# evanwporter/SparseCholesky

Hardware: AMD Instinct MI355X
Metric: numeric-factorization fp64 GFLOP/s (F=sum colcount^2) (higher is better)
Workload: dtype f64

## Files before the change

sparsecholesky_amd/csrc/kernels.hip:

```cpp
#include <hip/hip_runtime.h>

#include <cstdint>
#include <type_traits>

#include "kernels.hpp"

namespace sc {

typedef double double4_t __attribute__((ext_vector_type(4)));

__device__ __forceinline__ void report_fail(int32_t* info, const int32_t* post, int32_t col_internal) {
    atomicMin(info, (post ? post[col_internal] : col_internal) + 1);
}

__device__ __forceinline__ int bnd_at(const int32_t* b, int k, int mbc) {
    const int klo = b[0], khi = b[1];
    return k <= klo ? b[2] : (k >= khi ? mbc : b[2 + k - klo]);
}

__device__ __forceinline__ int lower_bound_i32(const int32_t* a, int n, int v) {
    int lo = 0, hi = n;
    while (lo < hi) {
        int mid = (lo + hi) >> 1;
        if (a[mid] < v)
// ... 677 lines not shown
        }
    }
}

template <int NP, int J>
__device__ __forceinline__ void td_steps(double (&a)[NP], double (&Ld)[4][4], double (&rc)[4], int& bad, int& fail,
                                         double* raw, double* lv, int i) {
    if constexpr (J < NP) {
        __builtin_amdgcn_sched_barrier(0);
        if (bad < 4) fail = min(fail, J + bad);
        const bool below = i >= J + 4;
        double l[4];
#pragma unroll
        for (int k = 0; k < 4; ++k) {
            double x = below ? a[J + k] : 0.0;
#pragma unroll
            for (int t = 0; t < k; ++t) x = fma(-l[t], Ld[k][t], x);
            l[k] = x * rc[k];
        }
        wave_lds_sync();
        *reinterpret_cast<double2*>(lv + 4 * i) = make_double2(l[0], l[1]);
        *reinterpret_cast<double2*>(lv + 4 * i + 2) = make_double2(l[2], l[3]);
        wave_lds_sync();
#pragma unroll
        for (int c = 0; c < 4; ++c) {
            double v = below ? l[c] : a[J + c];
#pragma unroll
            for (int r = c; r < 4; ++r) v = i == J + r ? Ld[r][c] : v;
            a[J + c] = v;
        }
        auto update = [&](int jj) {
            const double2 x01 = *reinterpret_cast<const double2*>(lv + 4 * jj);
            const double2 x23 = *reinterpret_cast<const double2*>(lv + 4 * jj + 2);
            double x = a[jj];
            x = fma(-l[0], x01.x, x);
            x = fma(-l[1], x01.y, x);
            x = fma(-l[2], x23.x, x);
            x = fma(-l[3], x23.y, x);
            a[jj] = x;
        };
        if constexpr (J + 4 < NP && !SC_TD_LA) {
#pragma unroll
            for (int jj = J + 4; jj < NP; ++jj) update(jj);
            wave_lds_sync();
            *reinterpret_cast<double2*>(raw + 4 * i) = make_double2(a[J + 4], a[J + 5]);
            *reinterpret_cast<double2*>(raw + 4 * i + 2) = make_double2(a[J + 6], a[J + 7]);
            wave_lds_sync();
            td_factor_d(raw, J + 4, Ld, rc, bad);
        }
        if constexpr (J + 4 < NP && SC_TD_LA) {
#pragma unroll
            for (int jj = J + 4; jj < J + 8; ++jj) update(jj);
            wave_lds_sync();
            *reinterpret_cast<double2*>(raw + 4 * i) = make_double2(a[J + 4], a[J + 5]);
            *reinterpret_cast<double2*>(raw + 4 * i + 2) = make_double2(a[J + 6], a[J + 7]);
            wave_lds_sync();
            double Dn[4][4], Ln[4][4], rn[4];
            int bn = 4;
#pragma unroll
            for (int r = 0; r < 4; ++r) {
                const double2 x01 = *reinterpret_cast<const double2*>(raw + 4 * (J + 4 + r));
                const double2 x23 = *reinterpret_cast<const double2*>(raw + 4 * (J + 4 + r) + 2);
                Dn[r][0] = x01.x;
                Dn[r][1] = x01.y;
                Dn[r][2] = x23.x;
                Dn[r][3] = x23.y;
            }
            auto pivot = [&](int c) {
                double dd = Dn[c][c];
#pragma unroll
                for (int t = 0; t < c; ++t) dd = fma(-Ln[c][t], Ln[c][t], dd);
                if (!(dd > 0.0)) bn = min(bn, c);
                rn[c] = rsqrt_f64(dd);
                Ln[c][c] = dd * rn[c];
#pragma unroll
                for (int r = c + 1; r < 4; ++r) {
                    double x = Dn[r][c];
#pragma unroll
                    for (int t = 0; t < c; ++t) x = fma(-Ln[r][t], Ln[c][t], x);
                    Ln[r][c] = x * rn[c];
                }
            };
            constexpr int GW = NP > 48 ? 4 : 8;
            constexpr int NG = (NP - J - 8 + GW - 1) / GW;
#pragma unroll
            for (int g = 0; g < NG; ++g) {
                if (g < 4) pivot(g);
#pragma unroll
                for (int u = 0; u < GW; ++u)
                    if (J + 8 + GW * g + u < NP) update(J + 8 + GW * g + u);
                __builtin_amdgcn_sched_barrier(0);
            }
#pragma unroll
            for (int c = NG; c < 4; ++c) pivot(c);
#pragma unroll
            for (int r = 0; r < 4; ++r) {
                rc[r] = rn[r];
#pragma unroll
                for (int c = 0; c < 4; ++c) Ld[r][c] = Ln[r][c];
            }
            bad = bn;
        }
        td_steps<NP, J + 4>(a, Ld, rc, bad, fail, raw, lv, i);
    }
}

template <int NP>
__global__ __launch_bounds__(64) void tiny_dense_kernel(DevPlan P, TinyPlan T, int n, const double* __restrict__ Ax) {
    __shared__ __attribute__((aligned(16))) double raw[NP * 4];
    __shared__ __attribute__((aligned(16))) double lv[NP * 4];
    __shared__ int po[NP * 64];
    const int i = threadIdx.x;
    int2 q[NP];
#pragma unroll
    for (int j = 0; j < NP; ++j) q[j] = T.a[j * 64 + i];
#pragma unroll
    for (int j = 0; j < NP; ++j) po[j * 64 + i] = q[j].y;
    double a[NP];
    int fail = n;
    double Ld[4][4], rc[4];
    int bad;
#pragma unroll
    for (int j = 0; j < NP; ++j) {
#if SC_TD_BUF
        a[j] = buf_ld(buf_rsrc(Ax, (uint32_t)T.nax * 8u), q[j].x >= 0 ? q[j].x * 8 : BUF_DEAD, 0);
#else
        a[j] = q[j].x >= 0 ? Ax[q[j].x] : 0.0;
#endif
    }
#pragma unroll
    for (int j = 0; j < NP; ++j) a[j] = (i == j && i >= n) ? 1.0 : a[j];
    if (SC_TD_PROBE != 1) {
        wave_lds_sync();
        *reinterpret_cast<double2*>(raw + 4 * i) = make_double2(a[0], a[1]);
        *reinterpret_cast<double2*>(raw + 4 * i + 2) = make_double2(a[2], a[3]);
        wave_lds_sync();
        td_factor_d(raw, 0, Ld, rc, bad);
        td_steps<NP, 0>(a, Ld, rc, bad, fail, raw, lv, i);
    }
    if (fail > n) fail = n;
#pragma unroll
    for (int j = 0; j < NP; ++j) {
        const int o = po[j * 64 + i];
#if SC_TD_BUF
        buf_st(a[j], buf_rsrc(P.panel_pool, (uint32_t)T.npan * 8u), o >= 0 ? o * 8 : BUF_DEAD, 0);
#else
        if (o >= 0) P.panel_pool[o] = a[j];
#endif
    }
    int32_t nat = fail < n ? (P.post ? P.post[fail] : fail) : 0x7f7f7f7f;
    if (fail < n) {
        __shared__ double rec[NP * 64];
#pragma unroll
        for (int j = 0; j < NP; ++j) {
            const int2 q = T.a[j * 64 + i];
            rec[j * 64 + i] = q.x >= 0 ? Ax[q.x] : 0.0;
        }
        for (int j = 0; j < n; ++j) {
            wave_lds_sync();
            const double d = rec[j * 64 + j];
            const bool ok = d > 0.0;
            if (!ok) nat = min(nat, P.post ? P.post[j] : j);
            const double l = (ok && i > j) ? rec[j * 64 + i] / sqrt(d) : 0.0;
            lv[i] = l;
            wave_lds_sync();
            for (int k = j + 1; k < n; ++k)
                if (i >= k) rec[k * 64 + i] -= l * lv[k];
        }
    }
    if (i == 0) {
        if (T.host_info) {
            const int32_t st = fail < n ? nat + 1 : 0x7f7f7f7f;
            P.info[0] = st;
            __hip_atomic_store(T.host_info, st, __ATOMIC_RELEASE, __HIP_MEMORY_SCOPE_SYSTEM);
        } else if (fail < n) {
            atomicMin(P.info, nat + 1);
        }
    }
}

hipError_t launch_tiny_dense(const DevPlan& P, const TinyPlan& T, int n, const double* Ax, hipStream_t st) {
    if (n <= 0) return hipSuccess;
    if (n > TINY_DENSE_N || T.na != tiny_dense_np(n) * 64) return hipErrorInvalidValue;
    if ((int64_t)T.nax * 8 >= BUF_DEAD || (int64_t)T.npan * 8 >= BUF_DEAD) return hipErrorInvalidValue;
    if (n <= 16)
        hipLaunchKernelGGL(tiny_dense_kernel<16>, dim3(1), dim3(64), 0, st, P, T, n, Ax);
    else if (n <= 32)
        hipLaunchKernelGGL(tiny_dense_kernel<32>, dim3(1), dim3(64), 0, st, P, T, n, Ax);
    else if (n <= 48)
        hipLaunchKernelGGL(tiny_dense_kernel<48>, dim3(1), dim3(64), 0, st, P, T, n, Ax);
    else
        hipLaunchKernelGGL(tiny_dense_kernel<64>, dim3(1), dim3(64), 0, st, P, T, n, Ax);
    return hipGetLastError();
}

__global__ __launch_bounds__(256) void chain_init_kernel(DevPlan P, ChainPlan C, int first,
                                                          const double* __restrict__ Ax) {
    extern __shared__ double F[];
    const ChainDesc d = C.desc[first + blockIdx.x];
    small_assemble(P, d.s, d.c0, d.w, d.m, Ax, F, d.sp);
    const int tot = (d.m * (d.m + 1)) >> 1;
    double* out = C.init + d.init_off;
    for (int idx = threadIdx.x; idx < tot; idx += 256) out[idx] = F[idx];
}

#ifndef SC_CHAIN_DB
#define SC_CHAIN_DB 1
#endif
constexpr int CHAIN_IMG = (128 * 129 / 2 + CHAIN_NT - 1) / CHAIN_NT;
__global__ __launch_bounds__(CHAIN_NT) void front_chain_kernel(DevPlan P, ChainPlan C, int first, int count, int fsz) {
    extern __shared__ double F[];
    __shared__ __attribute__((aligned(16))) double colbuf[2 * 4 * COLB];
    __shared__ ChainDesc ds[CHAIN_MAXF];
    const int tid = threadIdx.x;
    for (int i = tid; i < count; i += CHAIN_NT) ds[i] = C.desc[first + i];
    lds_barrier();
    double img[CHAIN_IMG];
    int nbi, nbj;
    uint32_t nrr, nrc;
    auto prefetch = [&](int f) {
        const ChainDesc& d = ds[f];
        const int tot = (d.m * (d.m + 1)) >> 1;
        const double* src = C.init + d.init_off;
#pragma unroll
        for (int q = 0; q < CHAIN_IMG; ++q) {
            const int idx = tid + CHAIN_NT * q;
            img[q] = idx < tot ? src[idx] : 0.0;
        }
        const int T = (d.m + 3) >> 2;
        nbi = nbj = -1;
        if (tid < T * (T + 1) / 2) tile_map(tid, T, (d.w + 3) >> 2, nbi, nbj);
        nrr = nbi >= 0 ? C.relp[d.relp_off + nbi] : 0u;
        nrc = nbi >= 0 ? C.relp[d.relp_off + nbj] : 0u;
    };
    auto Fb = [&](int f) { return SC_CHAIN_DB ? F + (f & 1) * fsz : F; };
    auto put = [&](int f) {
        const int tot = (ds[f].m * (ds[f].m + 1)) >> 1;
        double* Fd = Fb(f);
#pragma unroll
        for (int q = 0; q < CHAIN_IMG; ++q) {
            const int idx = tid + CHAIN_NT * q;
            if (idx < tot) Fd[idx] = img[q];
        }
    };
    int cbi, cbj;
    uint32_t crr, crc;
    auto take = [&]() {
        cbi = nbi;
        cbj = nbj;
        crr = nrr;
        crc = nrc;
    };
    prefetch(0);
    put(0);
    take();
    if (count > 1) prefetch(1);
    lds_barrier();
    for (int i = 0; i < count; ++i) {
        uint64_t* stamp = C.stamps ? C.stamps + 8 * (first + i) : nullptr;
        if (stamp && tid == 0) stamp[0] = __builtin_amdgcn_s_memtime();
        const ChainDesc d = ds[i];
        const int m = d.m, w = d.w;
        SmallRegs<1> R;
        R.bi[0] = cbi;
        R.bj[0] = cbj;
        const uint32_t rr = crr, rc = crc;
        small_load<1>(R, Fb(i), m);
        if (!SC_CHAIN_DB) lds_barrier();
        if (stamp && tid == 0) stamp[1] = __builtin_amdgcn_s_memtime();
        const bool has_parent = i + 1 < count;
        if (has_parent) {
            put(i + 1);
            take();
            if (i + 2 < count) prefetch(i + 2);
        }
        if (stamp && tid == 0) stamp[2] = __builtin_amdgcn_s_memtime();
        small_steps<1>(R, colbuf, w, P.info, P.post, d.c0);
        if (w == 0) lds_barrier();
        if (stamp && tid == 0) stamp[3] = __builtin_amdgcn_s_memtime();
        small_store_panel<1>(R, P.panel_pool + d.panel_off, m, w);
        if (m > w && R.bi[0] >= 0 && 4 * R.bi[0] + 3 >= w) {
            if (!has_parent) {
                small_store_cb<1>(R, P.cb_pool + d.cb_off, m, w);
            } else {
                const int mp = ds[i + 1].m;
                double* Fp = Fb(i + 1);
#pragma unroll
                for (int r = 0; r < 4; ++r)
#pragma unroll
                    for (int c = 0; c < 4; ++c) {
                        const int ii = 4 * R.bi[0] + r, jj = 4 * R.bj[0] + c;
                        const int pr = (rr >> (8 * r)) & 255, pc = (rc >> (8 * c)) & 255;
                        if (jj >= w && ii >= jj && ii < m) Fp[pk_col(mp, pc) + pr - pc] += R.v[0][r * 4 + c];
                    }
            }
        }
        lds_barrier();
        if (stamp && tid == 0) stamp[4] = __builtin_amdgcn_s_memtime();
    }
}

#include "panel_gen.inc"

__global__ __launch_bounds__(256) void potrf_tiles_kernel(DevPlan P, const int2* __restrict__ tasks) {
    __shared__ __attribute__((aligned(16))) double colbuf[2 * 4 * COLB];
    const int2 t = tasks[blockIdx.x];
    const int s = t.x, k0 = t.y;
    const int c0 = P.sn_start[s];
    const int w = P.sn_start[s + 1] - c0;
    const int m = P.sn_m[s];
    const int nb = min(PNB, w - k0);
    double* blk = P.panel_pool + P.panel_off[s] + (int64_t)k0 * m + k0;
    SmallRegs<1> R;
    small_tiles<1>(R, nb, nb);
#pragma unroll
    for (int r = 0; r < 4; ++r)
#pragma unroll
        for (int c = 0; c < 4; ++c) {
            const int i = 4 * R.bi[0] + r, j = 4 * R.bj[0] + c;
            R.v[0][r * 4 + c] = (R.bi[0] >= 0 && i < nb && i >= j) ? blk[(int64_t)j * m + i] : 0.0;
        }
    if (SC_POTRF_FAST)
        small_steps1_fast(R, colbuf, nb, P.info, P.post, c0 + k0);
    else
        small_steps<1>(R, colbuf, nb, P.info, P.post, c0 + k0);
    if (R.bi[0] < 0) return;
#pragma unroll
    for (int r = 0; r < 4; ++r)
#pragma unroll
        for (int c = 0; c < 4; ++c) {
            const int i = 4 * R.bi[0] + r, j = 4 * R.bj[0] + c;
            if (i < nb && i >= j) blk[(int64_t)j * m + i] = R.v[0][r * 4 + c];
        }
}

__device__ __forceinline__ void trsm_partial(double* pan, int m, int k0, int nb, int r0, int nrows, double* Lc,
                                             double* invd) {
    constexpr int LD = PNB + 2;
    const int tid = threadIdx.x;
    const double* blk = pan + (int64_t)k0 * m + k0;
    for (int idx = tid; idx < PNB * PNB; idx += TRSM_ROWS) {
        const int q = idx % PNB, j = idx / PNB;
        const double v = (q < nb && j < nb && j <= q) ? blk[(int64_t)j * m + q] : 0.0;
        Lc[j * LD + q] = v;
        if (q == j) invd[j] = (j < nb) ? 1.0 / v : 0.0;
    }
    __syncthreads();
    const int row = r0 + tid;
    const bool live = row < m && tid < nrows;
    double* xs = pan + (int64_t)k0 * m + (live ? row : r0);
    double r[PNB];
#pragma unroll
    for (int c = 0; c < PNB; ++c) r[c] = (live && c < nb) ? xs[(int64_t)c * m] : 0.0;
    trsm_steps<0>(r, Lc, invd, nb);
    if (live) {
#pragma unroll
        for (int c = 0; c < PNB; ++c)
            if (c < nb) xs[(int64_t)c * m] = r[c];
    }
}

__global__ __launch_bounds__(TRSM_ROWS) void trsm_partial_kernel(DevPlan P, const TrsmTask* __restrict__ tasks) {
    __shared__ double Lc[PNB * (PNB + 2)];
    __shared__ double invd[PNB];
    const TrsmTask t = tasks[blockIdx.x];
    const int s = t.s, k0 = t.k0, r0 = t.r0;
    const int c0 = P.sn_start[s];
    const int w = P.sn_start[s + 1] - c0;
    const int m = P.sn_m[s];
    trsm_partial(P.panel_pool + P.panel_off[s], m, k0, min(PNB, w - k0), r0, min(TRSM_ROWS, t.r1 - r0), Lc, invd);
}

template <int PRE>
__global__ __launch_bounds__(TRSM_ROWS) void trsm_panel_g_kernel(DevPlan P, const TrsmTask* __restrict__ tasks,
                                                                 int32_t* __restrict__ arrive) {
    static_assert(TRSM_ROWS == 256, "the fused POTRF maps 4 x 4 tiles onto 256 threads");
    __shared__ double2 S[TRSM64_STREAM / 2];
    __shared__ __attribute__((aligned(16))) double colbuf[2 * 4 * COLB];
    __shared__ int s_last;
    const TrsmTask t = tasks[blockIdx.x];
    const int s = t.s, k0 = t.k0, r0 = t.r0, r1 = t.r1;
    const int tid = threadIdx.x;
    const int c0 = P.sn_start[s];
    const int w = P.sn_start[s + 1] - c0;
    const int m = P.sn_m[s];
    const int nb = min(PNB, w - k0);
    double* pan = P.panel_pool + P.panel_off[s];
    if (nb < PNB) return;
    double* blk = pan + (int64_t)k0 * m + k0;
    double* Sd = reinterpret_cast<double*>(S);
    SmallRegs<1> R;
    small_tiles<1>(R, PNB, PNB);
#pragma unroll
    for (int r = 0; r < 4; ++r)
#pragma unroll
        for (int c = 0; c < 4; ++c) {
            const int i = 4 * R.bi[0] + r, j = 4 * R.bj[0] + c;
            R.v[0][r * 4 + c] = (R.bi[0] >= 0 && i >= j) ? blk[(int64_t)j * m + i] : 0.0;
        }
    if constexpr (PRE == 2) {
        if (R.bi[0] >= 0) {
#pragma unroll
            for (int r = 0; r < 4; ++r)
#pragma unroll
                for (int c = 0; c < 4; ++c) {
                    const int i = 4 * R.bi[0] + r, j = 4 * R.bj[0] + c;
                    if (i >= j) Sd[PNB * j - j * (j - 1) / 2 + (i - j)] = (i == j) ? 1.0 / R.v[0][r * 4 + c] : R.v[0][r * 4 + c];
                }
        }
        const int row = r0 + tid;
        const __amdgpu_buffer_rsrc_t rs = buf_rsrc(pan + (int64_t)k0 * m, (uint32_t)m * PNB * 8u);
        const int voff = row < r1 ? row * 8 : BUF_DEAD;
        double r[PNB];
#pragma unroll
        for (int c = 0; c < PNB; ++c) r[c] = buf_ld(rs, voff, c * m * 8);
        __syncthreads();
        trsm64_full(r, S);
#pragma unroll
        for (int c = 0; c < PNB; ++c) buf_st(r[c], rs, voff, c * m * 8);
        return;
    }
    if (SC_POTRF_FAST)
        small_steps1_fast(R, colbuf, PNB, P.info, P.post, c0 + k0);
    else
        small_steps<1>(R, colbuf, PNB, P.info, P.post, c0 + k0);
    if (R.bi[0] >= 0) {
#pragma unroll
        for (int r = 0; r < 4; ++r)
#pragma unroll
            for (int c = 0; c < 4; ++c) {
                const int i = 4 * R.bi[0] + r, j = 4 * R.bj[0] + c;
                if (i >= j) Sd[PNB * j - j * (j - 1) / 2 + (i - j)] = (i == j) ? 1.0 / R.v[0][r * 4 + c] : R.v[0][r * 4 + c];
            }
    }
    const int row = r0 + tid;
    const __amdgpu_buffer_rsrc_t rs = buf_rsrc(pan + (int64_t)k0 * m, (uint32_t)m * PNB * 8u);
    const int voff = row < r1 ? row * 8 : BUF_DEAD;
    double r[PNB];
#pragma unroll
    for (int c = 0; c < PNB; ++c) r[c] = buf_ld(rs, voff, c * m * 8);
    __syncthreads();
    if (tid == 0) {
        const int k1 = k0 + PNB;
        const int nwg = (max(r1, k1 + 1) - k1 + TRSM_ROWS - 1) / TRSM_ROWS;
        const int old = __hip_atomic_fetch_add(arrive + (t.ctr - 1), 1, __ATOMIC_RELAXED, __HIP_MEMORY_SCOPE_AGENT);
        s_last = old == nwg - 1;
        if (old == nwg - 1) __hip_atomic_store(arrive + (t.ctr - 1), 0, __ATOMIC_RELAXED, __HIP_MEMORY_SCOPE_AGENT);
    }
    __syncthreads();
    if (s_last && R.bi[0] >= 0) {
#pragma unroll
        for (int rr = 0; rr < 4; ++rr)
#pragma unroll
            for (int c = 0; c < 4; ++c) {
                const int i = 4 * R.bi[0] + rr, j = 4 * R.bj[0] + c;
                if (i >= j) blk[(int64_t)j * m + i] = R.v[0][rr * 4 + c];
            }
    }
    trsm64_full(r, S);
#pragma unroll
    for (int c = 0; c < PNB; ++c) buf_st(r[c], rs, voff, c * m * 8);
}

#ifndef SC_PROBE_NOGATHER
#define SC_PROBE_NOGATHER 0
#endif
#ifndef SC_PROBE_NOK
#define SC_PROBE_NOK 0
#endif
template <int BT, int WM, int WN, int BK = 16, int GR = 64>
__device__ __forceinline__ void syrk_gather_epilogue(const GemmTask& T, const int64_t* __restrict__ gblk,
                                                     const GSeg* __restrict__ gseg, int row0, int col0,
                                                     double4_t (&acc)[BT / WM / 16][BT / WN / 16], double* smem) {
    constexpr int NW = WM * WN, NT = 64 * NW;
    constexpr int RTM = BT / WM / 16, RTN = BT / WN / 16;
    constexpr int GLD = GR + 1;
    constexpr int GQ = BT == 64 ? (GR == 32 ? 8 : 64 / NW) : SC_GATHER_Q;
    constexpr int SB = BT == 64 ? 4 : 1;
    constexpr int OPS = 2 * 2 * BK * (BT + 16);
    static_assert(BT * GLD <= OPS, "gather chunk fits the operand LDS");
    const int tid = threadIdx.x, lane = tid & 63, wid = tid >> 6;
    const int wr = wid / WN, wc = wid % WN;
    const int w = T.gw;
    const int mb = T.M;
    const int nb = (mb + 63) >> 6;
    const int64_t* __restrict__ blk = gblk + T.gb;
    const GSeg* __restrict__ seg = gseg;
    double* G = smem;
    double* __restrict__ C = T.C;
    const int64_t ldc = T.ldc;
    const __amdgpu_buffer_rsrc_t rc = buf_rsrc(C + (int64_t)col0 * ldc, (uint32_t)(min(BT, T.N - col0) * ldc * 8));
#pragma unroll 1
    for (int h = 0; h < BT / GR; ++h) {
        const int r0 = row0 + h * GR;
        const int rb = r0 >> 6;
        if (h) __syncthreads();
        for (int e = tid; e < BT * GLD; e += NT) G[e] = 0.0;
        __syncthreads();
        const int cb1 = min(min(nb, rb + 1), (col0 + BT) >> 6);
        for (int cbk = col0 >> 6; !SC_PROBE_NOGATHER && r0 < mb && cbk < cb1; ++cbk) {
            const int64_t bi = (int64_t)rb * (rb + 1) / 2 + cbk;
            const int64_t p0 = blk[bi], p1 = blk[bi + 1];
            for (int64_t pb = p0; pb < p1; pb += SB) {
                int prw[SB], pcl[SB];
#pragma unroll
                for (int q = 0; q < SB; ++q) {
                    prw[q] = -1;
                    pcl[q] = -1;
                    if (pb + q < p1) {
                        const GSeg& g = seg[pb + q];
                        const int ic = g.ilo + lane, jl = g.jlo + lane;
                        if (ic < g.ihi) prw[q] = g.rel[ic] - w - r0;
                        if (jl < g.jhi) pcl[q] = g.rel[jl] - w - col0;
                    }
                }
#pragma unroll
                for (int q = 0; q < SB; ++q) {
                    if (pb + q >= p1) break;
                    const GSeg& g = seg[pb + q];
                    const int ic = g.ilo + lane;
                    const int prow = prw[q] < GR ? prw[q] : -1;
                    const int mbc = g.mbc;
                    const double* __restrict__ cb = g.cb;
                    uint64_t mask = __ballot(pcl[q] >= 0 && pcl[q] % NW == wid);
                    while (mask) {
                        int jc[GQ], pc[GQ];
#pragma unroll
                        for (int u = 0; u < GQ; ++u) {
                            const int b = mask ? __builtin_ctzll(mask) : -1;
                            jc[u] = b < 0 ? -1 : g.jlo + b;
                            pc[u] = b < 0 ? 0 : __builtin_amdgcn_readlane(pcl[q], b);
                            mask &= mask - 1;
                        }
                        double v[GQ];
                        bool ok[GQ];
#pragma unroll
                        for (int u = 0; u < GQ; ++u) {
                            ok[u] = jc[u] >= 0 && prow >= 0 && ic >= jc[u];
                            const __amdgpu_buffer_rsrc_t rs = buf_rsrc(cb + (int64_t)max(jc[u], 0) * mbc, (uint32_t)mbc * 8u);
                            v[u] = buf_ld(rs, ok[u] ? ic * 8 : BUF_DEAD, 0);
                        }
#pragma unroll
                        for (int u = 0; u < GQ; ++u)
                            if (ok[u]) G[pc[u] * GLD + prow] += v[u];
                    }
                }
            }
        }
        __syncthreads();
        static_assert(GR % (BT / WM) == 0, "a wave's rows lie in one chunk");
        if ((wr * (BT / WM)) / GR == h) {
#pragma unroll
            for (int a = 0; a < RTM; ++a)
#pragma unroll
                for (int b = 0; b < RTN; ++b)
#pragma unroll
                    for (int r = 0; r < 4; ++r) {
                        const int lr = wr * (BT / WM) + a * 16 + MFMA_F64_ROW(lane, r);
                        const int lc = wc * (BT / WN) + b * 16 + (lane & 15);
                        G[lc * GLD + (lr - h * GR)] -= acc[a][b][r];
                    }
        }
        __syncthreads();
#pragma unroll 4
        for (int e = tid; e < BT * GR; e += NT) {
            const int lr = e % GR, lc = e / GR;
            const int gi = r0 + lr, gj = col0 + lc;
            const bool live = gi < T.M && gi >= gj && gj < T.N;
            buf_st(G[lc * GLD + lr], rc, live ? (int)((gi + (int64_t)(gj - col0) * ldc) * 8) : BUF_DEAD, 0);
        }
    }
}

template <int BT, int WM, int WN, int BK = 16, int GR = 64>
__device__ __forceinline__ void syrk_rmw_epilogue(const GemmTask& T, int row0, int col0,
                                                  double4_t (&acc)[BT / WM / 16][BT / WN / 16], double* smem) {
    constexpr int NW = WM * WN, NT = 64 * NW;
    constexpr int RTM = BT / WM / 16, RTN = BT / WN / 16;
    constexpr int GLD = GR + 1;
    constexpr int OPS = 2 * 2 * BK * (BT + 16);
    static_assert(BT * GLD <= OPS, "chunk fits the operand LDS");
    static_assert(GR % (BT / WM) == 0, "a wave's rows lie in one chunk");
    const int tid = threadIdx.x, lane = tid & 63, wid = tid >> 6;
    const int wr = wid / WN, wc = wid % WN;
    double* G = smem;
    const int64_t ldc = T.ldc;
    const __amdgpu_buffer_rsrc_t rc = buf_rsrc(T.C + (int64_t)col0 * ldc, (uint32_t)(min(BT, T.N - col0) * ldc * 8));
#pragma unroll 1
    for (int h = 0; h < BT / GR; ++h) {
        const int r0 = row0 + h * GR;
        if (h) __syncthreads();
#pragma unroll 4
        for (int e = tid; e < BT * GR; e += NT) {
            const int lr = e % GR, lc = e / GR;
            const int gi = r0 + lr, gj = col0 + lc;
            const bool live = gi < T.M && gi >= gj && gj < T.N;
            G[lc * GLD + lr] = buf_ld(rc, live ? (int)((gi + (int64_t)(gj - col0) * ldc) * 8) : BUF_DEAD, 0);
        }
        __syncthreads();
        if ((wr * (BT / WM)) / GR == h) {
#pragma unroll
            for (int a = 0; a < RTM; ++a)
#pragma unroll
                for (int b = 0; b < RTN; ++b)
#pragma unroll
                    for (int r = 0; r < 4; ++r) {
                        const int lr = wr * (BT / WM) + a * 16 + MFMA_F64_ROW(lane, r);
                        const int lc = wc * (BT / WN) + b * 16 + (lane & 15);
                        G[lc * GLD + (lr - h * GR)] -= acc[a][b][r];
                    }
        }
        __syncthreads();
#pragma unroll 4
        for (int e = tid; e < BT * GR; e += NT) {
            const int lr = e % GR, lc = e / GR;
            const int gi = r0 + lr, gj = col0 + lc;
            const bool live = gi < T.M && gi >= gj && gj < T.N;
            buf_st(G[lc * GLD + lr], rc, live ? (int)((gi + (int64_t)(gj - col0) * ldc) * 8) : BUF_DEAD, 0);
        }
    }
}

template <int BT, int WM, int WN, int BK = 16>
__device__ __forceinline__ void mfma_kloop(const double* __restrict__ A, int64_t lda, int K, int M, int N, int row0,
                                           int col0, double4_t (&acc)[BT / WM / 16][BT / WN / 16], double* smem) {
    static_assert(BK == 16 || BK == 8, "four-deep k sub-steps of the MFMA");
    constexpr int NT = 64 * WM * WN;
    constexpr int LDT = BT + 16;
    constexpr int RTM = BT / WM / 16, RTN = BT / WN / 16;
    double(*As)[BK * LDT] = reinterpret_cast<double(*)[BK * LDT]>(smem);
    double(*Bs)[BK * LDT] = reinterpret_cast<double(*)[BK * LDT]>(smem + 2 * BK * LDT);
    const int tid = threadIdx.x;
    const int lane = tid & 63;
    const int wid = tid >> 6;
    const int wr = wid / WN, wc = wid % WN;
    constexpr int PER = BT * BK / NT;
    double ra[PER], rb[PER];
    auto gload = [&](int k0) {
        const __amdgpu_buffer_rsrc_t rs = buf_rsrc(A + (int64_t)k0 * lda, (uint32_t)(min(BK, K - k0) * lda * 8));
#pragma unroll
        for (int q = 0; q < PER; ++q) {
            const int e = tid + q * NT;
            const int r = e % BT, kk = e / BT;
            const int gr = row0 + r, gc = col0 + r;
            ra[q] = buf_ld(rs, gr < M ? (int)((gr + kk * lda) * 8) : BUF_DEAD, 0);
            rb[q] = buf_ld(rs, gc < N ? (int)((gc + kk * lda) * 8) : BUF_DEAD, 0);
        }
    };
    auto sstore = [&](int buf) {
#pragma unroll
        for (int q = 0; q < PER; ++q) {
            const int e = tid + q * NT;
            const int r = e % BT, kk = e / BT;
            As[buf][kk * LDT + r] = ra[q];
            Bs[buf][kk * LDT + r] = rb[q];
        }
    };

    const int nk = (K + BK - 1) / BK;
    auto stage = [&](int kt, auto last) {
        constexpr bool LAST = decltype(last)::value;
        const int cur = kt & 1;
        if (!LAST) gload((kt + 1) * BK);
        double av[2][RTM], bv[2][RTN];
        auto lread = [&](int kk, int slot) {
            const int krow = kk + (lane >> 4);
#pragma unroll
            for (int a = 0; a < RTM; ++a)
                av[slot][a] = As[cur][krow * LDT + wr * (BT / WM) + a * 16 + (lane & 15)];
#pragma unroll
            for (int b = 0; b < RTN; ++b)
                bv[slot][b] = Bs[cur][krow * LDT + wc * (BT / WN) + b * 16 + (lane & 15)];
        };
        lread(0, 0);
#pragma unroll
        for (int kk = 0; kk < BK; kk += 4) {
            const int slot = (kk / 4) & 1;
            if (kk + 4 < BK) lread(kk + 4, slot ^ 1);
#pragma unroll
            for (int a = 0; a < RTM; ++a)
#pragma unroll
                for (int b = 0; b < RTN; ++b)
                    acc[a][b] = __builtin_amdgcn_mfma_f64_16x16x4f64(av[slot][a], bv[slot][b], acc[a][b], 0, 0, 0);
            if (!LAST && kk == BK - 8) sstore(cur ^ 1);
        }
        __syncthreads();
    };
    gload(0);
    sstore(0);
    __syncthreads();
    for (int kt = 0; kt + 1 < nk; ++kt) stage(kt, std::false_type {});
    if (nk > 0) stage(nk - 1, std::true_type {});
}

template <int BK>
__device__ __forceinline__ void panel_prefactor(const GemmTask& T, int32_t* info, const int32_t* post,
                                                double* smem) {
    static_assert(2 * 2 * BK * (64 + 16) >= 64 * 65 / 2, "the packed diagonal block fits the operand LDS");
    double4_t acc[2][2];
#pragma unroll
    for (int a = 0; a < 2; ++a)
#pragma unroll
        for (int b = 0; b < 2; ++b) acc[a][b] = (double4_t){0.0, 0.0, 0.0, 0.0};
    mfma_kloop<64, 2, 2, BK>(T.A, T.lda, T.K, T.M, T.N, 0, 0, acc, smem);
    const int tid = threadIdx.x, lane = tid & 63, wid = tid >> 6;
    const int wr = wid >> 1, wc = wid & 1;
    const int64_t ldc = T.ldc;
    double* __restrict__ F = smem;
    const __amdgpu_buffer_rsrc_t rc = buf_rsrc(T.C, (uint32_t)(64 * ldc * 8));
    double cv[2][2][4];
#pragma unroll
    for (int a = 0; a < 2; ++a)
#pragma unroll
        for (int b = 0; b < 2; ++b)
#pragma unroll
            for (int r = 0; r < 4; ++r) {
                const int gi = wr * 32 + a * 16 + MFMA_F64_ROW(lane, r), gj = wc * 32 + b * 16 + (lane & 15);
                cv[a][b][r] = buf_ld(rc, gi >= gj ? (int)((gi + (int64_t)gj * ldc) * 8) : BUF_DEAD, 0);
            }
#pragma unroll
    for (int a = 0; a < 2; ++a)
#pragma unroll
        for (int b = 0; b < 2; ++b)
#pragma unroll
            for (int r = 0; r < 4; ++r) {
                const int gi = wr * 32 + a * 16 + MFMA_F64_ROW(lane, r), gj = wc * 32 + b * 16 + (lane & 15);
                if (gi >= gj) F[pk_col(64, gj) + gi - gj] = cv[a][b][r] - acc[a][b][r];
            }
    __syncthreads();
    SmallRegs<1> R;
    small_tiles<1>(R, PNB, PNB);
    small_load<1>(R, F, PNB);
    __syncthreads();
    small_steps1_fast(R, smem, PNB, info, post, T.pf);
    if (R.bi[0] < 0) return;
#pragma unroll
    for (int r = 0; r < 4; ++r)
#pragma unroll
        for (int c = 0; c < 4; ++c) {
            const int i = 4 * R.bi[0] + r, j = 4 * R.bj[0] + c;
            if (i >= j) T.C[(int64_t)j * ldc + i] = R.v[0][r * 4 + c];
        }
}

template <int BT, int WM, int WN, int TAG, int EPI, int LEAN = 0, int PF = 0>
__device__ __forceinline__ void syrk_tile_body(const GemmTask* __restrict__ tasks, const int2* __restrict__ tiles,
                                               int bidx, const int64_t* __restrict__ gblk,
                                               const GSeg* __restrict__ gseg, int32_t* info = nullptr,
                                               const int32_t* post = nullptr) {
    constexpr int BK = LEAN ? 8 : 16;
    constexpr int LDT = BT + 16;
    constexpr int RTM = BT / WM / 16, RTN = BT / WN / 16;
    __shared__ __attribute__((aligned(16))) double smem[2 * 2 * BK * LDT];

    const int2 tl = tiles[bidx];
    const GemmTask T = tasks[tl.x];
    if constexpr (PF) {
        static_assert(BT == 64 && WM == 2 && WN == 2 && TAG == 0, "pre-factor on 64 x 64 panel-update tiles");
        if (tl.y < 0) {
            panel_prefactor<BK>(T, info, post, smem);
            return;
        }
    }
    const int ti = tl.y >> 16, tj = tl.y & 0xffff;
    const int row0 = ti * BT, col0 = tj * BT;

    const int wid = threadIdx.x >> 6;
    if (wid >= WM * WN / 2) __builtin_amdgcn_s_setprio(1);

    double4_t acc[RTM][RTN];
#pragma unroll
    for (int a = 0; a < RTM; ++a)
#pragma unroll
        for (int b = 0; b < RTN; ++b) acc[a][b] = (double4_t){0.0, 0.0, 0.0, 0.0};
    if (!(SC_PROBE_NOK && TAG == 1 && T.gs >= 0)) mfma_kloop<BT, WM, WN, BK>(T.A, T.lda, T.K, T.M, T.N, row0, col0, acc, smem);

    if constexpr (TAG == 1) {
        if (T.gs >= 0) {
            syrk_gather_epilogue<BT, WM, WN, BK, LEAN ? 32 : 64>(T, gblk, gseg, row0, col0, acc, smem);
            return;
        }
    }
    syrk_rmw_epilogue<BT, WM, WN, BK, LEAN ? 32 : 64>(T, row0, col0, acc, smem);
}

template <int BT, int WM, int WN, int TAG, int EPI, int LEAN = 0, int PF = 0>
__global__ __launch_bounds__(64 * WM * WN, LEAN ? (TAG ? 5 : 6) : 1) void syrk_mfma_kernel(const GemmTask* __restrict__ tasks,
                                                                  const int2* __restrict__ tiles,
                                                                  const int64_t* __restrict__ gblk,
                                                                  const GSeg* __restrict__ gseg, int32_t* info,
                                                                  const int32_t* post) {
    syrk_tile_body<BT, WM, WN, TAG, EPI, LEAN, PF>(tasks, tiles, blockIdx.x, gblk, gseg, info, post);
}

static int small_kt(int maxm) {
    const int T = (maxm + 3) / 4;
    return (T * (T + 1) / 2 + 255) / 256;
}

hipError_t launch_front_small(const DevPlan& P, const int32_t* nodes, int count, int maxm, bool seq,
                              const double* Ax, hipStream_t st) {
    if (count <= 0) return hipSuccess;
    const size_t lds = (size_t)maxm * (maxm + 1) / 2 * sizeof(double);
    const int kt = small_kt(maxm);
    const dim3 grid(seq ? 1 : count);
    const int sq = seq ? count : 0;
    if (kt <= 1)
        hipLaunchKernelGGL(front_small_kernel<1>, grid, dim3(256), lds, st, P, nodes, Ax, sq);
    else if (kt == 2)
        hipLaunchKernelGGL(front_small_kernel<2>, grid, dim3(256), lds, st, P, nodes, Ax, sq);
    else
        hipLaunchKernelGGL(front_small_kernel<3>, grid, dim3(256), lds, st, P, nodes, Ax, sq);
    return hipGetLastError();
}

hipError_t launch_front_chain(const DevPlan& P, const ChainPlan& C, int first, int count, int maxm,
                              const double* Ax, hipStream_t st) {
    if (count <= 0) return hipSuccess;
    if (count > CHAIN_MAXF || maxm > 128) return hipErrorInvalidValue;
    const int fsz = maxm * (maxm + 1) / 2;
    const size_t lds = (size_t)fsz * sizeof(double);
    hipLaunchKernelGGL(chain_init_kernel, dim3(count), dim3(256), lds, st, P, C, first, Ax);
    hipLaunchKernelGGL(front_chain_kernel, dim3(1), dim3(CHAIN_NT), (SC_CHAIN_DB ? 2 : 1) * lds, st, P, C, first, count,
                       fsz);
    return hipGetLastError();
}

hipError_t launch_assemble_large(const DevPlan& P, const int2* tasks, int count, const double* Ax,
                                 hipStream_t st, bool tiled, const int2* lim) {
    if (count <= 0) return hipSuccess;
    if (tiled)
        hipLaunchKernelGGL(assemble_tile_kernel, dim3(count), dim3(256), 0, st, P, tasks, Ax, lim);
    else
        hipLaunchKernelGGL(assemble_cols_kernel, dim3(count), dim3(256), 0, st, P, tasks, Ax);
    return hipGetLastError();
}

hipError_t launch_potrf_diag(const DevPlan& P, const int2* tasks, int count, hipStream_t st) {
    if (count <= 0) return hipSuccess;
    hipLaunchKernelGGL(potrf_tiles_kernel, dim3(count), dim3(256), 0, st, P, tasks);
    return hipGetLastError();
}

hipError_t launch_trsm_panel(const DevPlan& P, const TrsmTask* tasks, int count, hipStream_t st, bool partial,
                             int32_t* arrive, int pre) {
    if (count <= 0) return hipSuccess;
    if (partial)
        hipLaunchKernelGGL(trsm_partial_kernel, dim3(count), dim3(TRSM_ROWS), 0, st, P, tasks);
    else if (pre == 2)
        hipLaunchKernelGGL(trsm_panel_g_kernel<2>, dim3(count), dim3(TRSM_ROWS), 0, st, P, tasks, arrive);
    else
        hipLaunchKernelGGL(trsm_panel_g_kernel<0>, dim3(count), dim3(TRSM_ROWS), 0, st, P, tasks, arrive);
    return hipGetLastError();
}

template <int TAG, int EPI>
static void launch_syrk_t(const GemmTask* tasks, const int2* tiles, int n, int bt, hipStream_t st, GatherTab gt,
                          bool lean) {
    if (bt == 64 && lean)
        hipLaunchKernelGGL((syrk_mfma_kernel<64, 2, 2, TAG, EPI, 1>), dim3(n), dim3(256), 0, st, tasks, tiles, gt.blk,
                           gt.seg, gt.info, gt.post);
    else if (bt == 128)
        hipLaunchKernelGGL((syrk_mfma_kernel<128, 2, 4, TAG, EPI>), dim3(n), dim3(512), 0, st, tasks, tiles, gt.blk,
                           gt.seg, gt.info, gt.post);
    else
        hipLaunchKernelGGL((syrk_mfma_kernel<64, 2, 2, TAG, EPI>), dim3(n), dim3(256), 0, st, tasks, tiles, gt.blk,
                           gt.seg, gt.info, gt.post);
}

hipError_t launch_syrk(const GemmTask* tasks, const int2* tiles, int total_tiles, int bt, int tag, hipStream_t st,
                       int epi, GatherTab gt, bool lean, bool pf) {
    if (total_tiles <= 0) return hipSuccess;
    if (pf) {
        if (bt != 64 || tag) return hipErrorInvalidValue;
        hipLaunchKernelGGL((syrk_mfma_kernel<64, 2, 2, 0, 1, 0, 1>), dim3(total_tiles), dim3(256), 0, st, tasks, tiles,
                           gt.blk, gt.seg, gt.info, gt.post);
        return hipGetLastError();
    }
    if (tag)
        epi ? launch_syrk_t<1, 1>(tasks, tiles, total_tiles, bt, st, gt, lean)
            : launch_syrk_t<1, 0>(tasks, tiles, total_tiles, bt, st, gt, lean);
    else
        epi ? launch_syrk_t<0, 1>(tasks, tiles, total_tiles, bt, st, gt, lean)
            : launch_syrk_t<0, 0>(tasks, tiles, total_tiles, bt, st, gt, lean);
    return hipGetLastError();
}

__global__ void fill_random_kernel(double* p, int64_t n) {
    for (int64_t i = blockIdx.x * (int64_t)blockDim.x + threadIdx.x; i < n; i += (int64_t)gridDim.x * blockDim.x) {
        uint64_t x = (uint64_t)i * 0x9E3779B97F4A7C15ull;
        x ^= x >> 31;
        x *= 0xBF58476D1CE4E5B9ull;
        x ^= x >> 29;
        p[i] = (double)(x >> 11) * (2.0 / 9007199254740992.0) - 1.0;
    }
}

hipError_t launch_fill_random(double* p, int64_t n, hipStream_t st) {
    hipLaunchKernelGGL(fill_random_kernel, dim3(1024), dim3(256), 0, st, p, n);
    return hipGetLastError();
}

__global__ void stamp_kernel(uint64_t* slot) { *slot = __builtin_amdgcn_s_memrealtime(); }

__global__ void status_publish_kernel(int32_t* info, int32_t* host) {
    const int32_t v = __hip_atomic_load(info, __ATOMIC_RELAXED, __HIP_MEMORY_SCOPE_AGENT);
    __hip_atomic_store(info, 0x7f7f7f7f, __ATOMIC_RELAXED, __HIP_MEMORY_SCOPE_AGENT);
    __hip_atomic_store(host, v, __ATOMIC_RELEASE, __HIP_MEMORY_SCOPE_SYSTEM);
}

hipError_t launch_status_publish(int32_t* info, int32_t* host, hipStream_t st) {
    hipLaunchKernelGGL(status_publish_kernel, dim3(1), dim3(1), 0, st, info, host);
    return hipGetLastError();
}

__global__ void hwid_kernel(uint32_t* out, int spin) {
    if (threadIdx.x == 0) {
        out[2 * blockIdx.x] = __builtin_amdgcn_s_getreg((31 << 11) | 4);
        out[2 * blockIdx.x + 1] = __builtin_amdgcn_s_getreg((15 << 11) | 20);
    }
    const uint64_t t0 = __builtin_amdgcn_s_memrealtime();
    while (__builtin_amdgcn_s_memrealtime() - t0 < (uint64_t)spin) __builtin_amdgcn_s_sleep(8);
}

hipError_t launch_hwid(uint32_t* out, int nwg, int threads, int spin, hipStream_t st) {
    hipLaunchKernelGGL(hwid_kernel, dim3(nwg), dim3(threads), 0, st, out, spin);
    return hipGetLastError();
}

hipError_t launch_stamp(uint64_t* slot, hipStream_t st) {
    hipLaunchKernelGGL(stamp_kernel, dim3(1), dim3(1), 0, st, slot);
    return hipGetLastError();
}

__global__ __launch_bounds__(256) void copy2d_kernel(const Copy2D* __restrict__ descs, const int2* __restrict__ tiles,
                                                     int unpack) {
    const int2 t = tiles[blockIdx.x];
    const Copy2D d = descs[t.x];
    const int lane = threadIdx.x & 63, wid = threadIdx.x >> 6;
    const int j0 = t.y & 0xffff, r0 = (t.y >> 16) * COPY_ROWS;
    const int j1 = min(d.cols, j0 + COPY_COLS), r1 = min(d.rows, r0 + COPY_ROWS);
    for (int j = j0 + wid; j < j1; j += 4) {
        const double* __restrict__ src = unpack ? d.b + (int64_t)j * d.rows : d.a + (int64_t)j * d.lda;
        double* __restrict__ dst = unpack ? d.a + (int64_t)j * d.lda : d.b + (int64_t)j * d.rows;
        for (int r = r0 + lane; r < r1; r += 64 * 8) {
            double v[8];
#pragma unroll
            for (int u = 0; u < 8; ++u) v[u] = r + 64 * u < r1 ? src[r + 64 * u] : 0.0;
#pragma unroll
            for (int u = 0; u < 8; ++u)
                if (r + 64 * u < r1) dst[r + 64 * u] = v[u];
        }
    }
}

hipError_t launch_copy2d(const Copy2D* descs, const int2* tiles, int count, bool unpack, hipStream_t st) {
    if (count <= 0) return hipSuccess;
    hipLaunchKernelGGL(copy2d_kernel, dim3(count), dim3(256), 0, st, descs, tiles, unpack ? 1 : 0);
    return hipGetLastError();
}

template <int NACC>
__global__ __launch_bounds__(256) void mfma_peak_kernel(double* out, int iters) {
    double4_t acc[NACC];
#pragma unroll
    for (int j = 0; j < NACC; ++j) acc[j] = (double4_t){0.0, 0.0, 0.0, 0.0};
    const double a = 1.0 + threadIdx.x * 1e-9, b = 1.0 - blockIdx.x * 1e-9;
    for (int i = 0; i < iters; i += 16) {
#pragma unroll
        for (int u = 0; u < 16; ++u)
#pragma unroll
            for (int j = 0; j < NACC; ++j) acc[j] = __builtin_amdgcn_mfma_f64_16x16x4f64(a, b, acc[j], 0, 0, 0);
    }
    double s = 0.0;
#pragma unroll
    for (int j = 0; j < NACC; ++j) s += acc[j][0] + acc[j][1] + acc[j][2] + acc[j][3];
    if (s == 1234.5) out[blockIdx.x] = s;
}

hipError_t launch_mfma_peak(double* out, int blocks, int iters, int nacc, hipStream_t st) {
    if (nacc == 16)
        hipLaunchKernelGGL((mfma_peak_kernel<16>), dim3(blocks), dim3(256), 0, st, out, iters);
    else if (nacc == 8)
        hipLaunchKernelGGL((mfma_peak_kernel<8>), dim3(blocks), dim3(256), 0, st, out, iters);
    else if (nacc == 2)
        hipLaunchKernelGGL((mfma_peak_kernel<2>), dim3(blocks), dim3(256), 0, st, out, iters);
    else
        hipLaunchKernelGGL((mfma_peak_kernel<4>), dim3(blocks), dim3(256), 0, st, out, iters);
    return hipGetLastError();
}

__global__ __launch_bounds__(64) void solve_inv_kernel(SolvePlan P, const int2* __restrict__ tasks) {
    __shared__ double2 S[TRSM64_STREAM / 2];
    __shared__ double Lc[PNB * (PNB + 2)];
    __shared__ double invd[PNB];
    const int2 t = tasks[blockIdx.x];
    const int s = t.x, k0 = t.y;
    const int lane = threadIdx.x;
    const int c0 = P.sn_start[s];
    const int w = P.sn_start[s + 1] - c0;
    const int m = P.sn_m[s];
    const int nb = min(PNB, w - k0);
    double* blk = const_cast<double*>(P.panel_pool) + P.panel_off[s] + (int64_t)k0 * m + k0;
    double r[PNB];
    {
#pragma unroll
        for (int j = 0; j < PNB; ++j) r[j] = (j < nb && lane < nb && lane >= j) ? blk[(int64_t)j * m + lane] : 0.0;
    }
    if (nb == PNB) {
        double* Sd = reinterpret_cast<double*>(S);
#pragma unroll
        for (int j = 0; j < PNB; ++j)
            if (lane >= j) Sd[PNB * j - j * (j - 1) / 2 + (lane - j)] = lane == j ? 1.0 / r[j] : r[j];
    } else {
        constexpr int LD = PNB + 2;
#pragma unroll
        for (int j = 0; j < PNB; ++j) {
            Lc[j * LD + lane] = r[j];
            if (lane == j) invd[j] = j < nb ? 1.0 / r[j] : 0.0;
        }
    }
    __syncthreads();
#pragma unroll
    for (int c = 0; c < PNB; ++c) r[c] = c == lane ? 1.0 : 0.0;
    if (nb == PNB)
        trsm64_full(r, S);
    else
        trsm_steps<0>(r, Lc, invd, nb);
#pragma unroll
    for (int c = 0; c < PNB; ++c)
        if (lane < c && c < nb) blk[(int64_t)c * m + lane] = r[c];
}

__global__ __launch_bounds__(256) void solve_inv2_kernel(SolvePlan P, const int2* __restrict__ tasks) {
    __shared__ double Xa[PNB][PNB + 1], Bm[PNB][PNB + 1], Xb[PNB][PNB + 1];
    const int2 t = tasks[blockIdx.x];
    const int s = t.x, k0 = t.y;
    const int tid = threadIdx.x;
    const int c0 = P.sn_start[s];
    const int w = P.sn_start[s + 1] - c0;
    const int m = P.sn_m[s];
    const int nbb = min(SOLVE_NB, w - k0) - PNB;
    double* blk = const_cast<double*>(P.panel_pool) + P.panel_off[s] + (int64_t)k0 * m + k0;
    const double* blkb = blk + (int64_t)PNB * m + PNB;
#pragma unroll
// ... 2140 lines not shown
```

Before: 58150.

## Replace register-tile 64x64 POTRF with LDS-staged blocked factorization using MFMA updates

Adds a blocked 64x64 Cholesky that stages the diagonal block into padded LDS. One wave factors each 16-column panel with lane shuffles, and all four waves apply the trailing updates with f64 MFMA. This path replaces the older 4x4 register-tile small_steps factorization in the full-block POTRF kernel, the fused POTRF+TRSM panel kernel and the GEMM pre-factor epilogue. It aims to cut the long serial per-column sync chain of the old POTRF. In exchange it uses more LDS per block, and most waves sit idle during each panel step.

```diff
diff --git a/sparsecholesky_amd/csrc/kernels.hip b/sparsecholesky_amd/csrc/kernels.hip
--- a/sparsecholesky_amd/csrc/kernels.hip
+++ b/sparsecholesky_amd/csrc/kernels.hip
@@ -1003,8 +1003,105 @@
 
 #include "panel_gen.inc"
 
+constexpr int POTRF_LD = PNB + 16;
+#ifndef SC_POTRF_STAMP
+#define SC_POTRF_STAMP(i)
+#endif
+__device__ __forceinline__ void potrf64_blocked(double* Cm, int32_t* info, const int32_t* post, int c0) {
+    constexpr int LD = POTRF_LD;
+    const int tid = threadIdx.x, lane = tid & 63, wid = tid >> 6;
+    int bad = PNB;
+    SC_POTRF_STAMP(0);
+#pragma unroll
+    for (int q = 0; q < 4; ++q) {
+        const int k0 = 16 * q;
+        if (wid == 0 && lane < PNB - k0) {
+            double* col = Cm + k0 * LD + k0 + lane;
+            double x[16];
+#pragma unroll
+            for (int c = 0; c < 16; ++c) x[c] = col[c * LD];
+#pragma unroll
+            for (int j = 0; j < 16; ++j) {
+                const double d = readlane_f64(x[j], j);
+                if (!(d > 0.0)) bad = min(bad, k0 + j);
+                const double rc = rsqrt_f64(d);
+                x[j] *= rc;
+#pragma unroll
+                for (int k = j + 1; k < 16; ++k) x[k] = fma(-x[j], readlane_f64(x[j], k), x[k]);
+            }
+#pragma unroll
+            for (int c = 0; c < 16; ++c) col[c * LD] = x[c];
+        }
+        SC_POTRF_STAMP(2 * q + 1);
+        if (q == 3) break;
+        lds_barrier();
+        const int n = 3 - q;
+        for (int t = wid; t < n * (n + 1) / 2; t += 4) {
+            int c = 0, rem = t;
+            while (rem >= n - c) {
+                rem -= n - c;
+                ++c;
+            }
+            const int i0 = 16 * (q + 1 + c + rem), j0 = 16 * (q + 1 + c);
+            const int lr = lane & 15, lk = lane >> 4;
+            double4_t acc;
+#pragma unroll
+            for (int r = 0; r < 4; ++r) acc[r] = Cm[(j0 + lk + 4 * r) * LD + i0 + lr];
+            double av[4], bv[4];
+#pragma unroll
+            for (int kk = 0; kk < 4; ++kk) {
+                av[kk] = -Cm[(k0 + 4 * kk + lk) * LD + j0 + lr];
+                bv[kk] = Cm[(k0 + 4 * kk + lk) * LD + i0 + lr];
+            }
+#pragma unroll
+            for (int kk = 0; kk < 4; ++kk) acc = __builtin_amdgcn_mfma_f64_16x16x4f64(av[kk], bv[kk], acc, 0, 0, 0);
+#pragma unroll
+            for (int r = 0; r < 4; ++r) Cm[(j0 + lk + 4 * r) * LD + i0 + lr] = acc[r];
+        }
+        lds_barrier();
+        SC_POTRF_STAMP(2 * q + 2);
+    }
+    if (bad < PNB && tid == 0) report_fail(info, post, c0 + bad);
+}
+
+__device__ __forceinline__ void potrf64_stage(double* Cm, const double* __restrict__ blk, int64_t ld) {
+    const int i = threadIdx.x & 63, jq = threadIdx.x >> 6;
+    double v[PNB / 4];
+#pragma unroll
+    for (int u = 0; u < PNB / 4; ++u) {
+        const int j = jq + 4 * u;
+        v[u] = i >= j ? blk[(int64_t)j * ld + i] : 0.0;
+    }
+#pragma unroll
+    for (int u = 0; u < PNB / 4; ++u) Cm[(jq + 4 * u) * POTRF_LD + i] = v[u];
+}
+
+__device__ __forceinline__ void potrf64_unstage(const double* Cm, double* __restrict__ blk, int64_t ld) {
+    const int i = threadIdx.x & 63, jq = threadIdx.x >> 6;
+#pragma unroll
+    for (int u = 0; u < PNB / 4; ++u) {
+        const int j = jq + 4 * u;
+        if (i >= j) blk[(int64_t)j * ld + i] = Cm[j * POTRF_LD + i];
+    }
+}
+
+__device__ __forceinline__ void potrf64_stream(const double* Cm, double* Sd) {
+    const int i = threadIdx.x & 63, jq = threadIdx.x >> 6;
+    const double rd = 1.0 / Cm[i * POTRF_LD + i];
+#pragma unroll
+    for (int u = 0; u < PNB / 4; ++u) {
+        const int j = jq + 4 * u;
+        if (i >= j) {
+            const double v = Cm[j * POTRF_LD + i];
+            Sd[PNB * j - j * (j - 1) / 2 + (i - j)] = (i == j) ? rd : v;
+        }
+    }
+}
+
 __global__ __launch_bounds__(256) void potrf_tiles_kernel(DevPlan P, const int2* __restrict__ tasks) {
-    __shared__ __attribute__((aligned(16))) double colbuf[2 * 4 * COLB];
+    static_assert(PNB * POTRF_LD >= 2 * 4 * COLB, "the partial block's column buffer overlays the full block's image");
+    __shared__ __attribute__((aligned(16))) double Cm[PNB * POTRF_LD];
+    double* colbuf = Cm;
     const int2 t = tasks[blockIdx.x];
     const int s = t.x, k0 = t.y;
     const int c0 = P.sn_start[s];
@@ -1012,6 +1109,14 @@
     const int m = P.sn_m[s];
     const int nb = min(PNB, w - k0);
     double* blk = P.panel_pool + P.panel_off[s] + (int64_t)k0 * m + k0;
+    if (nb == PNB) {
+        potrf64_stage(Cm, blk, m);
+        lds_barrier();
+        potrf64_blocked(Cm, P.info, P.post, c0 + k0);
+        lds_barrier();
+        potrf64_unstage(Cm, blk, m);
+        return;
+    }
     SmallRegs<1> R;
     small_tiles<1>(R, nb, nb);
 #pragma unroll
@@ -1075,9 +1180,9 @@
 template <int PRE>
 __global__ __launch_bounds__(TRSM_ROWS) void trsm_panel_g_kernel(DevPlan P, const TrsmTask* __restrict__ tasks,
                                                                  int32_t* __restrict__ arrive) {
-    static_assert(TRSM_ROWS == 256, "the fused POTRF maps 4 x 4 tiles onto 256 threads");
+    static_assert(TRSM_ROWS == 256, "the fused POTRF runs on four waves");
     __shared__ double2 S[TRSM64_STREAM / 2];
-    __shared__ __attribute__((aligned(16))) double colbuf[2 * 4 * COLB];
+    __shared__ __attribute__((aligned(16))) double Cm[PRE == 2 ? 2 : PNB * POTRF_LD];
     __shared__ int s_last;
     const TrsmTask t = tasks[blockIdx.x];
     const int s = t.s, k0 = t.k0, r0 = t.r0, r1 = t.r1;
@@ -1090,16 +1195,22 @@
     if (nb < PNB) return;
     double* blk = pan + (int64_t)k0 * m + k0;
     double* Sd = reinterpret_cast<double*>(S);
-    SmallRegs<1> R;
-    small_tiles<1>(R, PNB, PNB);
-#pragma unroll
-    for (int r = 0; r < 4; ++r)
-#pragma unroll
-        for (int c = 0; c < 4; ++c) {
-            const int i = 4 * R.bi[0] + r, j = 4 * R.bj[0] + c;
-            R.v[0][r * 4 + c] = (R.bi[0] >= 0 && i >= j) ? blk[(int64_t)j * m + i] : 0.0;
-        }
     if constexpr (PRE == 2) {
+        SmallRegs<1> R;
+        small_tiles<1>(R, PNB, PNB);
+#pragma unroll
+        for (int r = 0; r < 4; ++r)
+#pragma unroll
+            for (int c = 0; c < 4; ++c) {
+                const int i = 4 * R.bi[0] + r, j = 4 * R.bj[0] + c;
+                R.v[0][r * 4 + c] = (R.bi[0] >= 0 && i >= j) ? blk[(int64_t)j * m + i] : 0.0;
+            }
+        const int row = r0 + tid;
+        const __amdgpu_buffer_rsrc_t rs = buf_rsrc(pan + (int64_t)k0 * m, (uint32_t)m * PNB * 8u);
+        const int voff = row < r1 ? row * 8 : BUF_DEAD;
+        double r[PNB];
+#pragma unroll
+        for (int c = 0; c < PNB; ++c) r[c] = buf_ld(rs, voff, c * m * 8);
         if (R.bi[0] >= 0) {
 #pragma unroll
             for (int r = 0; r < 4; ++r)
@@ -1109,37 +1220,23 @@
                     if (i >= j) Sd[PNB * j - j * (j - 1) / 2 + (i - j)] = (i == j) ? 1.0 / R.v[0][r * 4 + c] : R.v[0][r * 4 + c];
                 }
         }
-        const int row = r0 + tid;
-        const __amdgpu_buffer_rsrc_t rs = buf_rsrc(pan + (int64_t)k0 * m, (uint32_t)m * PNB * 8u);
-        const int voff = row < r1 ? row * 8 : BUF_DEAD;
-        double r[PNB];
-#pragma unroll
-        for (int c = 0; c < PNB; ++c) r[c] = buf_ld(rs, voff, c * m * 8);
         __syncthreads();
         trsm64_full(r, S);
 #pragma unroll
         for (int c = 0; c < PNB; ++c) buf_st(r[c], rs, voff, c * m * 8);
         return;
     }
-    if (SC_POTRF_FAST)
-        small_steps1_fast(R, colbuf, PNB, P.info, P.post, c0 + k0);
-    else
-        small_steps<1>(R, colbuf, PNB, P.info, P.post, c0 + k0);
-    if (R.bi[0] >= 0) {
-#pragma unroll
-        for (int r = 0; r < 4; ++r)
-#pragma unroll
-            for (int c = 0; c < 4; ++c) {
-                const int i = 4 * R.bi[0] + r, j = 4 * R.bj[0] + c;
-                if (i >= j) Sd[PNB * j - j * (j - 1) / 2 + (i - j)] = (i == j) ? 1.0 / R.v[0][r * 4 + c] : R.v[0][r * 4 + c];
-            }
-    }
+    potrf64_stage(Cm, blk, m);
     const int row = r0 + tid;
     const __amdgpu_buffer_rsrc_t rs = buf_rsrc(pan + (int64_t)k0 * m, (uint32_t)m * PNB * 8u);
     const int voff = row < r1 ? row * 8 : BUF_DEAD;
     double r[PNB];
 #pragma unroll
     for (int c = 0; c < PNB; ++c) r[c] = buf_ld(rs, voff, c * m * 8);
+    lds_barrier();
+    potrf64_blocked(Cm, P.info, P.post, c0 + k0);
+    lds_barrier();
+    potrf64_stream(Cm, Sd);
     __syncthreads();
     if (tid == 0) {
         const int k1 = k0 + PNB;
@@ -1149,15 +1246,7 @@
         if (old == nwg - 1) __hip_atomic_store(arrive + (t.ctr - 1), 0, __ATOMIC_RELAXED, __HIP_MEMORY_SCOPE_AGENT);
     }
     __syncthreads();
-    if (s_last && R.bi[0] >= 0) {
-#pragma unroll
-        for (int rr = 0; rr < 4; ++rr)
-#pragma unroll
-            for (int c = 0; c < 4; ++c) {
-                const int i = 4 * R.bi[0] + rr, j = 4 * R.bj[0] + c;
-                if (i >= j) blk[(int64_t)j * m + i] = R.v[0][rr * 4 + c];
-            }
-    }
+    if (s_last) potrf64_unstage(Cm, blk, m);
     trsm64_full(r, S);
 #pragma unroll
     for (int c = 0; c < PNB; ++c) buf_st(r[c], rs, voff, c * m * 8);
@@ -1397,7 +1486,7 @@
 template <int BK>
 __device__ __forceinline__ void panel_prefactor(const GemmTask& T, int32_t* info, const int32_t* post,
                                                 double* smem) {
-    static_assert(2 * 2 * BK * (64 + 16) >= 64 * 65 / 2, "the packed diagonal block fits the operand LDS");
+    static_assert(2 * 2 * BK * (64 + 16) >= PNB * POTRF_LD, "the diagonal block's image fits the operand LDS");
     double4_t acc[2][2];
 #pragma unroll
     for (int a = 0; a < 2; ++a)
@@ -1407,7 +1496,7 @@
     const int tid = threadIdx.x, lane = tid & 63, wid = tid >> 6;
     const int wr = wid >> 1, wc = wid & 1;
     const int64_t ldc = T.ldc;
-    double* __restrict__ F = smem;
+    double* F = smem;
     const __amdgpu_buffer_rsrc_t rc = buf_rsrc(T.C, (uint32_t)(64 * ldc * 8));
     double cv[2][2][4];
 #pragma unroll
@@ -1426,22 +1515,12 @@
 #pragma unroll
             for (int r = 0; r < 4; ++r) {
                 const int gi = wr * 32 + a * 16 + MFMA_F64_ROW(lane, r), gj = wc * 32 + b * 16 + (lane & 15);
-                if (gi >= gj) F[pk_col(64, gj) + gi - gj] = cv[a][b][r] - acc[a][b][r];
+                F[gj * POTRF_LD + gi] = gi >= gj ? cv[a][b][r] - acc[a][b][r] : 0.0;
             }
     __syncthreads();
-    SmallRegs<1> R;
-    small_tiles<1>(R, PNB, PNB);
-    small_load<1>(R, F, PNB);
-    __syncthreads();
-    small_steps1_fast(R, smem, PNB, info, post, T.pf);
-    if (R.bi[0] < 0) return;
-#pragma unroll
-    for (int r = 0; r < 4; ++r)
-#pragma unroll
-        for (int c = 0; c < 4; ++c) {
-            const int i = 4 * R.bi[0] + r, j = 4 * R.bj[0] + c;
-            if (i >= j) T.C[(int64_t)j * ldc + i] = R.v[0][r * 4 + c];
-        }
+    potrf64_blocked(F, info, post, T.pf);
+    lds_barrier();
+    potrf64_unstage(F, T.C, ldc);
 }
 
 template <int BT, int WM, int WN, int TAG, int EPI, int LEAN = 0, int PF = 0>
```

Measured after the change: 58550 (median of 6 runs). No clear change (+0.7%).
